# penn-pal-lab/robot_aware_control

Hardware: AMD Instinct MI355X
Metric: SVG train frames/sec + CEM candidate-rollouts/sec, 64x64 (higher is better)
Workload: dtype fp32 (conv operands as two fp16 parts = 22 significant bits, fp32 accumulate; see fp32_exact)

## Files before the change

include/rac_hip.h:

```cpp
#ifndef RAC_HIP_H
#define RAC_HIP_H

#include <stddef.h>
#include <stdint.h>

#ifdef __cplusplus
extern "C" {
#endif

#define RAC_OK 0
#define RAC_EINVAL (-1)
#define RAC_ELAUNCH (-2)

#define RAC_ABI_VERSION 12

int rac_version(void);
const char* rac_device_arch(void);
const char* rac_last_error(void);

enum {
  RAC_CONV_FWD = 0,
  RAC_CONV_DGRAD = 1,
  RAC_CONV_WGRAD = 2
};
// ... 169 lines not shown
int rac_reparam_head_bwd(const rac_grad_src* dz_srcs, int32_t n_srcs, const float* logvar, const float* eps,
                         const float* dmu_add, const float* dlogvar_add, float* dy, int64_t M, int32_t z,
                         uint32_t* dy_amax, void* stream);

int rac_reparam_fwd(const float* mu, const float* logvar, const float* eps, float* z, int64_t n, void* stream);
int rac_reparam_bwd(const float* dz, const float* logvar, const float* eps, float* dlogvar, int64_t n, void* stream);

int rac_pack_input(const float* img, const float* zmask, const float* mask, int32_t Cm, int32_t pad, float* packed,
                   int32_t B, int32_t HW, void* stream);
int rac_first_layer_fwd(const float* img, const float* zmask, const float* mask, int32_t Cm, const float* w,
                        const float* scale, const float* shift, int32_t act, float* out, uint32_t* out_amax,
                        int32_t amax_per_image, int32_t B, int32_t H, int32_t W, int32_t Cout, void* stream);
int rac_first_layer_fwd_split(const float* img, const float* zmask, const float* mask, int32_t Cm, const float* w,
                              const float* scale, const float* shift, int32_t act, float* out, uint32_t* out_amax,
                              int32_t amax_per_image, int32_t B, int32_t H, int32_t W, int32_t Cout, void* stream);
int rac_head_fwd(const float* x, const float* w_taps, const float* bias, float* y, int32_t B, int32_t H, int32_t W,
                 void* stream);
int rac_head_dgrad(const float* d, const float* w, float* dx, int32_t B, int32_t H, int32_t W, void* stream);
int rac_head_fwd_split(const float* x, const uint32_t* x_amax, int32_t amax_per_image, const float* w_taps,
                       const float* bias, float* y, int32_t B, int32_t H, int32_t W, void* stream);
int rac_thin_wgrad(const float* wide, const float* thin, int32_t thin_stride, int32_t Ct, float* parts, int32_t n_parts,
                   int32_t B, int32_t H, int32_t W, int32_t Cw, void* stream);
int rac_unpack_grad(const float* dpacked, int32_t C, const float* zmask, float* dimg, int32_t B, int32_t HW,
                    void* stream);
int rac_zero_region(const float* img, const float* mask, float* out, int32_t B, int32_t HW, void* stream);
int rac_composite_fwd(const float* x4, const float* prev, float* out, int32_t B, int32_t HW, void* stream);
int rac_composite_bwd(const float* dout, const float* x4, const float* prev, float* dx4, float* dprev, int32_t B,
                      int32_t HW, void* stream);
int rac_predict_frames(const float* x4, const float* prev, const float* target, const float* true_mask, float* pred,
                       uint8_t* gen_u8, uint8_t* true_u8, int64_t image_stride, int32_t n, int32_t nt, int32_t H,
                       int32_t W, void* stream);

typedef struct rac_image_job {
  int64_t frame_offset, mask_offset;
  int32_t Hs, Ws, top, left, th, tw;
  int32_t order[4];
  int32_t jitter;
// ... 135 lines not shown
```

robot_aware_control_amd/_lib.py:

```python
from __future__ import annotations

import ctypes as C
import os

import torch

_HERE = os.path.dirname(os.path.abspath(__file__))
LIB_PATH = os.environ.get("RAC_HIP_LIB") or os.path.join(_HERE, "librac_hip.so")

i32, i64, f32, vp = C.c_int32, C.c_int64, C.c_float, C.c_void_p


class ConvArgs(C.Structure):
    _fields_ = [
        ("mode", i32), ("B", i32), ("H", i32), ("W", i32), ("ksize", i32), ("Cin", i32), ("Cout", i32),
        ("act", i32), ("split_k", i32), ("accumulate", i32), ("a_split", i32), ("o_split", i32),
        ("slab_stride", i64),
        ("a0", vp), ("a1", vp), ("w", vp), ("out0", vp), ("out1", vp),
        ("bias", vp), ("scale", vp), ("shift", vp), ("stats", vp),
        ("stats_rows", i64), ("a0_up", i32), ("amax_per_image", i32),
    ]


WGRAD_MAX_STEPS = 16
# ... 104 lines not shown
    "rac_groupnorm_fwd": [vp, vp, vp, vp, vp, vp, i32, i32, i32, i32, f32, vp],
    "rac_norm_lstm_cell_fwd": [vp, vp, vp, vp, vp, vp, vp, vp, vp, vp, vp, vp, vp, vp, vp, vp, i32, i32, i32, f32, vp],
    "rac_groupnorm_bwd": [vp, vp, vp, vp, vp, vp, vp, vp, i32, i32, i32, i32, vp],
    "rac_norm_lstm_cell_bwd": [vp] * 25 + [i32, i32, i32, vp],
    "rac_lstm_out_fwd": [vp, vp, vp, i64, i32, vp],
    "rac_lstm_out_bwd": [vp, vp, vp, vp, vp, i64, i32, vp],
    "rac_lstm_core_bwd": [vp, vp, vp, vp, vp, vp, i64, i32, vp],
    "rac_grad_sum": [C.POINTER(GradSrc), i32, vp, i64, i32, vp, vp],
    "rac_lstm_cell_bwd_srcs": [C.POINTER(GradSrc), i32, vp, vp, vp, vp, vp, vp, i64, i32, vp, vp],
    "rac_reparam_head_bwd": [C.POINTER(GradSrc), i32, vp, vp, vp, vp, vp, i64, i32, vp, vp],
    "rac_reparam_fwd": [vp, vp, vp, vp, i64, vp],
    "rac_reparam_bwd": [vp, vp, vp, vp, i64, vp],
    "rac_pack_input": [vp, vp, vp, i32, i32, vp, i32, i32, vp],
    "rac_first_layer_fwd": [vp, vp, vp, i32, vp, vp, vp, i32, vp, vp, i32, i32, i32, i32, i32, vp],
    "rac_first_layer_fwd_split": [vp, vp, vp, i32, vp, vp, vp, i32, vp, vp, i32, i32, i32, i32, i32, vp],
    "rac_head_fwd": [vp, vp, vp, vp, i32, i32, i32, vp],
    "rac_head_dgrad": [vp, vp, vp, i32, i32, i32, vp],
    "rac_head_fwd_split": [vp, vp, i32, vp, vp, vp, i32, i32, i32, vp],
    "rac_thin_wgrad": [vp, vp, i32, i32, vp, i32, i32, i32, i32, i32, vp],
    "rac_unpack_grad": [vp, i32, vp, vp, i32, i32, vp],
    "rac_zero_region": [vp, vp, vp, i32, i32, vp],
    "rac_composite_fwd": [vp, vp, vp, i32, i32, vp],
    "rac_composite_bwd": [vp, vp, vp, vp, vp, i32, i32, vp],
    "rac_predict_frames": [vp, vp, vp, vp, vp, vp, vp, i64, i32, i32, i32, i32, vp],
    "rac_image_job_bytes": [],
    "rac_image_pipeline": [vp, vp, vp, vp, vp, i32, i32, i32, i32, vp],
    "rac_det_pack_fwd": [vp, i32, vp, i32, vp, vp, vp, i32, vp, vp, vp, i32, i32, i32, vp, vp],
    "rac_det_pack_bwd": [vp, i32, i32, vp, i32, vp, i32, vp, vp, vp, vp, vp, i32, i32, vp],
    "rac_copy_baseline": [vp, vp, vp, vp, i32, i32, vp],
    "rac_recon_loss_fwd": [i32, vp, vp, vp, f32, vp, vp, vp, i32, i32, vp],
    "rac_recon_loss_bwd": [i32, vp, vp, vp, f32, vp, vp, vp, vp, i32, i32, vp],
    "rac_kl_fwd": [vp, vp, vp, vp, i64, i32, vp, vp, vp],
    "rac_kl_bwd": [vp, vp, vp, vp, vp, i64, i32, vp, vp, vp, vp, vp],
    "rac_psnr_ssim": [vp, vp, vp, vp, vp, vp, i32, i32, i32, vp],
# ... 83 lines not shown
```

robot_aware_control_amd/csrc/rac_frame.hip:

```cpp
#include "rac_common.h"

namespace rac {

static inline int grid_for(long work_items) {
  long b = (work_items + 255) / 256;
  return (int)(b < 1 ? 1 : (b > 2048 ? 2048 : b));
}

__global__ void pack_input_kernel(const float* img, const float* zmask, const float* mask, int Cm, int pad,
                                  float* packed, int B, int HW) {
  const int C = 3 + Cm + pad;
  const long n = (long)B * HW;
  for (long i = blockIdx.x * (long)blockDim.x + threadIdx.x; i < n; i += (long)gridDim.x * blockDim.x) {
    long b = i / HW;
    int p = (int)(i - b * HW);
    const bool zero = zmask && zmask[i] != 0.f;
    float* o = packed + i * C;
#pragma unroll
    for (int c = 0; c < 3; ++c) {
      float v = img[(b * 3 + c) * HW + p];
      o[c] = zero ? v * 0.f : v;
    }
    for (int c = 0; c < Cm; ++c) o[3 + c] = mask[(b * Cm + c) * HW + p];
    for (int c = 0; c < pad; ++c) o[3 + Cm + c] = 0.f;
// ... 112 lines not shown
      for (int c4 = 0; c4 < 8; ++c4) {
        const f32x4 xv = *reinterpret_cast<const f32x4*>(xp + c4 * 4);
#pragma unroll
        for (int j = 0; j < 4; ++j)
#pragma unroll
          for (int c = 0; c < 4; ++c) acc[c] += xv[j] * wp[(c4 * 4 + j) * 4 + c];
      }
    }
  }
  f32x4 out;
#pragma unroll
  for (int c = 0; c < 4; ++c) out[c] = sigmoid_acc(acc[c]);
  *reinterpret_cast<f32x4*>(y + (((long)b * H + ty0 + py) * W + tx0 + px) * 4) = out;
}

template <int CT>
__global__ __launch_bounds__(256) void thin_wgrad_kernel(const float* wide, const float* thin, int ldt, float* part, int H,
                                                         int W, int n_tiles) {
  constexpr int TP = 18, NO = 9 * CT, NQ = (NO + 3) / 4;
  __shared__ float th[TP * TP][CT];
  const int tid = threadIdx.x, w = tid & 63, q = tid >> 6;
  const int tiles_x = W >> 4, tiles_img = (H >> 4) * tiles_x;
  float acc[NQ];
  int toff[NQ];
#pragma unroll
  for (int j = 0; j < NQ; ++j) {
    acc[j] = 0.f;
    const int o = min(q * NQ + j, NO - 1), tap = o / CT;
    toff[j] = ((tap / 3) * TP + tap % 3) * CT + (o - tap * CT);
  }
  const float* thf = &th[0][0];
  for (int tile = blockIdx.x; tile < n_tiles; tile += gridDim.x) {
    const int b = tile / tiles_img, ti = tile - b * tiles_img;
    const int ty0 = (ti / tiles_x) << 4, tx0 = (ti % tiles_x) << 4;
    __syncthreads();
    for (int i = tid; i < TP * TP * CT; i += 256) {
      const int pix = i / CT, t = i - pix * CT;
      const int y = ty0 + pix / TP - 1, x = tx0 + pix % TP - 1;
      th[pix][t] = ((unsigned)y < (unsigned)H && (unsigned)x < (unsigned)W)
                       ? thin[(((long)b * H + y) * W + x) * ldt + t] : 0.f;
    }
    __syncthreads();
    const float* wp = wide + (((long)b * H + ty0) * W + tx0) * 64 + w;
    for (int py = 0; py < 16; ++py) {
      float v[16];
#pragma unroll
      for (int px = 0; px < 16; ++px) v[px] = wp[((long)py * W + px) * 64];
#pragma unroll
      for (int px = 0; px < 16; ++px) {
        const float* tp = thf + (py * TP + px) * CT;
#pragma unroll
        for (int j = 0; j < NQ; ++j) acc[j] += v[px] * tp[toff[j]];
      }
    }
  }
  float* dst = part + (long)blockIdx.x * 64 * NO + (long)w * NO;
#pragma unroll
  for (int j = 0; j < NQ; ++j) {
    const int o = q * NQ + j;
    if (o < NO) dst[o] = acc[j];
  }
}

__global__ void unpack_grad_kernel(const float* dpacked, int C, const float* zmask, float* dimg, int B, int HW) {
  const long n = (long)B * HW;
  for (long i = blockIdx.x * (long)blockDim.x + threadIdx.x; i < n; i += (long)gridDim.x * blockDim.x) {
    long b = i / HW;
    int p = (int)(i - b * HW);
    const bool zero = zmask && zmask[i] != 0.f;
#pragma unroll
    for (int c = 0; c < 3; ++c) dimg[(b * 3 + c) * HW + p] = zero ? 0.f : dpacked[i * C + c];
  }
}

__global__ void zero_region_kernel(const float* img, const float* mask, float* out, int B, int HW) {
// ... 157 lines not shown
    }
  }
}

__device__ __forceinline__ float block_sum(float v, float* sh) {
  v = wave_sum(v);
  const int w = threadIdx.x >> 6, l = threadIdx.x & 63;
  __syncthreads();
  if (l == 0) sh[w] = v;
  __syncthreads();
  float t = 0.f;
  for (int k = 0; k < (int)(blockDim.x >> 6); ++k) t += sh[k];
  return t;
}

__global__ void recon_loss_sample_kernel(int kind, const float* pred, const float* target, const float* mask,
                                         float rw, float* per_sample, int HW) {
  __shared__ float sh[16];
  const int b = blockIdx.x;
  const long base = (long)b * 3 * HW;
  float s_main = 0.f, s_world_n = 0.f, s_rob2 = 0.f, s_rob_n = 0.f, s_world2 = 0.f;
  for (int p = threadIdx.x; p < HW; p += blockDim.x) {
    const bool rob = mask && mask[(long)b * HW + p] != 0.f;
    if (mask) {
      if (rob) s_rob_n += 3.f; else s_world_n += 3.f;
    }
#pragma unroll
    for (int c = 0; c < 3; ++c) {
      float d = target[base + (long)c * HW + p] - pred[base + (long)c * HW + p];
      if (mask) {
        if (rob) s_rob2 += d * d; else s_world2 += d * d;
      }
// ... 288 lines not shown
  RAC_REQUIRE(W % 16 == 0 && aligned16(d) && aligned16(w) && aligned16(dx), "rac_head_dgrad: W % 16 == 0, 16-byte aligned buffers");
  const long n_pix = (long)B * H * W;
  long per_block = ((n_pix + 511) / 512 + 15) / 16 * 16;
  if (per_block < 64) per_block = 64;
  const long blocks = (n_pix + per_block - 1) / per_block;
  RAC_REQUIRE(blocks < (1L << 31) && per_block < (1L << 31) && n_pix < (1L << 28) - 16, "rac_head_dgrad: too many pixels");
  hipLaunchKernelGGL(head_dgrad_kernel, dim3((unsigned)blocks), dim3(256), 0, ST(stream), reinterpret_cast<const float4*>(d),
                     reinterpret_cast<const float4*>(w), reinterpret_cast<float4*>(dx), H, W, n_pix, (int)per_block);
  return check_launch("rac_head_dgrad");
}

int rac_thin_wgrad(const float* wide, const float* thin, int32_t thin_stride, int32_t Ct, float* parts, int32_t n_parts,
                   int32_t B, int32_t H, int32_t W, int32_t Cw, void* stream) {
  RAC_REQUIRE(wide && thin && parts && B > 0 && H > 0 && W > 0 && Ct >= 1 && Ct <= 8 && thin_stride >= Ct && n_parts >= 1,
              "rac_thin_wgrad: bad args (1 <= Ct <= 8)");
  RAC_REQUIRE(Cw == 64 && H % 16 == 0 && W % 16 == 0, "rac_thin_wgrad: Cw 64, H and W multiples of 16");
  const int n_tiles = B * (H / 16) * (W / 16);
  RAC_REQUIRE(n_parts <= n_tiles, "rac_thin_wgrad: more parts than 16 x 16 tiles");
  typedef void (*fn_t)(const float*, const float*, int, float*, int, int, int);
  static const fn_t fns[8] = {thin_wgrad_kernel<1>, thin_wgrad_kernel<2>, thin_wgrad_kernel<3>, thin_wgrad_kernel<4>,
                              thin_wgrad_kernel<5>, thin_wgrad_kernel<6>, thin_wgrad_kernel<7>, thin_wgrad_kernel<8>};
  hipLaunchKernelGGL(fns[Ct - 1], dim3(n_parts), dim3(256), 0, ST(stream), wide, thin, thin_stride, parts, H, W, n_tiles);
  return check_launch("rac_thin_wgrad");
}

int rac_unpack_grad(const float* dpacked, int32_t C, const float* zmask, float* dimg, int32_t B, int32_t HW,
                    void* stream) {
  RAC_REQUIRE(dpacked && dimg && C >= 3 && B > 0 && HW > 0, "rac_unpack_grad: bad args");
  hipLaunchKernelGGL(unpack_grad_kernel, dim3(grid_for((long)B * HW)), dim3(256), 0, ST(stream), dpacked, C, zmask,
                     dimg, B, HW);
  return check_launch("rac_unpack_grad");
}

int rac_zero_region(const float* img, const float* mask, float* out, int32_t B, int32_t HW, void* stream) {
  RAC_REQUIRE(img && mask && out && B > 0 && HW > 0, "rac_zero_region: bad args");
  hipLaunchKernelGGL(zero_region_kernel, dim3(grid_for((long)B * 3 * HW)), dim3(256), 0, ST(stream), img, mask, out, B,
                     HW);
  return check_launch("rac_zero_region");
// ... 46 lines not shown
                  (!sheet || (aligned4(sheet) && aligned4(start_u8) && aligned4(goal_u8) && aligned4(goal_mask))),
              "rac_cem_rollout_sheet: 16-byte aligned float buffers, strides multiples of 4, 4-byte aligned uint8 buffers");
  const long quads = (long)(T + 1) * R * H * (W / 4);
  RAC_REQUIRE((long)H * W < (1L << 29) && quads < (1L << 40), "rac_cem_rollout_sheet: too many pixels");
  hipLaunchKernelGGL(cem_rollout_sheet_kernel, dim3(grid_for(quads)), dim3(256), 0, ST(stream), frames, (long)step_stride,
                     (long)cand_stride, rows, R, T, start_u8, goal_u8, G, goal_mask, obs, sheet, H, W);
  return check_launch("rac_cem_rollout_sheet");
}

int rac_recon_loss_fwd(int32_t kind, const float* pred, const float* target, const float* mask, float robot_weight,
                       const float* batch_weight, float* per_sample, float* out, int32_t B, int32_t HW, void* stream) {
  RAC_REQUIRE(kind >= 0 && kind <= 3 && pred && target && per_sample && out && B > 0 && HW > 0,
              "rac_recon_loss_fwd: bad args");
  RAC_REQUIRE(!((kind == RAC_LOSS_DONTCARE_L1 || kind == RAC_LOSS_DONTCARE_MSE) && !mask),
              "rac_recon_loss_fwd: dontcare loss needs a mask");
  hipLaunchKernelGGL(recon_loss_sample_kernel, dim3(B), dim3(256), 0, ST(stream), kind, pred, target, mask,
                     robot_weight, per_sample, HW);
  hipLaunchKernelGGL(recon_loss_final_kernel, dim3(1), dim3(256), 0, ST(stream), kind, per_sample, batch_weight,
                     mask != nullptr, out, B, HW);
  return check_launch("rac_recon_loss_fwd");
}

int rac_recon_loss_bwd(int32_t kind, const float* pred, const float* target, const float* mask, float robot_weight,
                       const float* batch_weight, const float* per_sample, const float* gout, float* dpred, int32_t B,
                       int32_t HW, void* stream) {
  RAC_REQUIRE(kind >= 0 && kind <= 3 && pred && target && per_sample && gout && dpred && B > 0 && HW > 0,
              "rac_recon_loss_bwd: bad args");
  RAC_REQUIRE(!((kind == RAC_LOSS_DONTCARE_L1 || kind == RAC_LOSS_DONTCARE_MSE) && !mask),
              "rac_recon_loss_bwd: dontcare loss needs a mask");
  hipLaunchKernelGGL(recon_loss_bwd_kernel, dim3(grid_for((long)B * 3 * HW)), dim3(256), 0, ST(stream), kind, pred,
                     target, mask, robot_weight, batch_weight, per_sample, gout, dpred, B, HW);
// ... 546 lines not shown
```

robot_aware_control_amd/csrc/rac_split16.hip:

```cpp
#include <math.h>
#include <stdlib.h>

#include <type_traits>

#include "rac_common.h"

namespace rac {

typedef _Float16 f16x8 __attribute__((ext_vector_type(8)));
typedef _Float16 f16x4 __attribute__((ext_vector_type(4)));
typedef unsigned int u32x4 __attribute__((ext_vector_type(4)));
typedef unsigned int u32x2 __attribute__((ext_vector_type(2)));
typedef __amdgpu_buffer_rsrc_t rsrc_t;

constexpr unsigned OOB = 0xFFFFFFF0u;
constexpr int SBN = 128, SBK = 32;

__device__ __forceinline__ const void* uniform_ptr(const void* p) {
  unsigned long long v = reinterpret_cast<unsigned long long>(p);
  unsigned lo = __builtin_amdgcn_readfirstlane((unsigned)v);
  unsigned hi = __builtin_amdgcn_readfirstlane((unsigned)(v >> 32));
  return reinterpret_cast<const void*>(((unsigned long long)hi << 32) | lo);
}
__device__ __forceinline__ rsrc_t make_rsrc(const void* p, unsigned bytes) {
// ... 707 lines not shown
    {
      const int py = tid >> 4, px = tid & 15;
      f32x4 o = b4;
#pragma unroll
      for (int tap = 0; tap < 9; ++tap) {
        const int ky = tap / 3, kx = tap - ky * 3;
        o += *reinterpret_cast<const f32x4*>(zs + (tap * H16_ZS + (py + 2 - ky) * H16_P + px + 2 - kx) * 4);
      }
#pragma unroll
      for (int c = 0; c < 4; ++c) o[c] = sigmoid_acc(o[c]);
      *reinterpret_cast<f32x4*>(y + (((long)b * H + ty0 + py) * W + tx0 + px) * 4) = o;
    }
  }
}

template <int CIN>
__global__ __launch_bounds__(256, 2) void first16_kernel(const float* __restrict__ img, const float* __restrict__ zmask,
                                                         const float* __restrict__ mask, const float* __restrict__ w,
                                                         const float* __restrict__ scale, const float* __restrict__ shift,
                                                         int act, float* __restrict__ out, unsigned* amax, int per_image,
                                                         int H, int W, int n_tiles) {
  constexpr int KK = 9 * CIN, KS = (KK + 31) / 32, TP = 18, TPW = 20, PL = TP * TPW;
  __shared__ float in_sh[CIN * PL];
  const int tid = threadIdx.x, lane = tid & 63, lr = lane & 15, lq = lane >> 4;
  const int wid = __builtin_amdgcn_readfirstlane(tid >> 6);
  f16x8 fw[4][KS][2];
  float osc[4][4], osh[4][4];
#pragma unroll
  for (int j = 0; j < 4; ++j) {
    const float* wr = w + (long)(16 * j + lr) * KK;
    float wv[KS][8], mx = 0.f;
#pragma unroll
    for (int s = 0; s < KS; ++s)
#pragma unroll
      for (int i = 0; i < 8; ++i) {
        const int k = 32 * s + 8 * lq + i;
        const float t = wr[min(k, KK - 1)];
        wv[s][i] = k < KK ? t : 0.f;
// ... 4 lines not shown
    const int kw = scale_exp(__builtin_bit_cast(unsigned, mx));
    const float sw = pow2f(kw);
#pragma unroll
    for (int s = 0; s < KS; ++s)
#pragma unroll
      for (int i = 0; i < 8; ++i) {
        const float v = wv[s][i] * sw;
        const _Float16 a = (_Float16)v;
        fw[j][s][0][i] = a;
        fw[j][s][1][i] = (_Float16)(v - (float)a);
      }
#pragma unroll
    for (int r = 0; r < 4; ++r) {
      const int kwr = __shfl(kw, 4 * lq + r);
      const int co = 16 * j + 4 * lq + r;
      osc[j][r] = (scale ? scale[co] : 1.f) * pow2f(-kwr);
      osh[j][r] = scale ? shift[co] : 0.f;
    }
  }
  int goff[KS][8];
#pragma unroll
  for (int s = 0; s < KS; ++s)
#pragma unroll
    for (int i = 0; i < 8; ++i) {
      const int k = min(32 * s + 8 * lq + i, KK - 1), tap = k / CIN, ci = k - tap * CIN;
      goff[s][i] = ci * PL + (tap / 3) * TPW + tap % 3;
    }
  const float slope = act == RAC_ACT_LEAKY02 ? 0.2f : 1.f;
  const int tiles_x = W >> 4, tiles_img = (H >> 4) * tiles_x;
  const long HW = (long)H * W;

  constexpr int NST = (CIN * TP * TP + 255) / 256;
// ... 58 lines not shown
        for (int i = 0; i < 8; ++i) {
          const float v = xv[s][i] * sa;
          const _Float16 a = (_Float16)v;
          fx[s][0][i] = a;
          fx[s][1][i] = (_Float16)(v - (float)a);
        }
      float* op = out + (((long)b * H + ty0 + py) * W + tx0 + lr) * 64 + 4 * lq;
#pragma unroll
      for (int j = 0; j < 4; ++j) {
        f32x4 acc = {0.f, 0.f, 0.f, 0.f};
#pragma unroll
        for (int s = 0; s < KS; ++s) acc = mma3(fw[j][s], fx[s], acc);
        f32x4 o;
#pragma unroll
        for (int r = 0; r < 4; ++r) {
          float v = fmaf(acc[r] * ia, osc[j][r], osh[j][r]);
          v = v > 0.f ? v : slope * v;
          mxo = max(mxo, absbits(v));
          o[r] = v;
        }
        *reinterpret_cast<f32x4*>(op + 16 * j) = o;
      }
    }
    if (amax) amax_commit_block(mxo, per_image ? amax + b : amax);
  }
}

template <int NV, int WM, int NT, int D, bool FAST = false, int KSF = 3>
__global__ __launch_bounds__(256, 2) void conv16_rows_kernel(Conv16P p) {
  constexpr int PF = KSF / 2, TAPSF = KSF * KSF;
  constexpr int WN = 4 / WM;
  constexpr int MB = 8 / WM;
  constexpr int NB = 2 * NT;
  constexpr int BNW = WN * NT * 32;
  extern __shared__ __attribute__((aligned(16))) unsigned char lds_raw[];
  const int tid = threadIdx.x;
  const int lane = tid & 63;
  const int wid = __builtin_amdgcn_readfirstlane(tid >> 6);
  const int lr = lane & 15, lq = lane >> 4;
// ... 1719 lines not shown
}

extern "C" int rac_first_layer_fwd_split(const float* img, const float* zmask, const float* mask, int32_t Cm, const float* w,
                                         const float* scale, const float* shift, int32_t act, float* out,
                                         uint32_t* out_amax, int32_t amax_per_image, int32_t B, int32_t H, int32_t W,
                                         int32_t Cout, void* stream) {
  RAC_REQUIRE(img && w && out && B > 0 && H > 0 && W > 0 && Cm >= 0 && Cm <= 5 && (Cm == 0 || mask),
              "rac_first_layer_fwd_split: bad args (3 image planes + at most 5 mask / heatmap planes)");
  RAC_REQUIRE(Cout == 64 && H % 16 == 0 && W % 16 == 0 && (scale == nullptr) == (shift == nullptr) && aligned16(out) &&
                  (act == RAC_ACT_NONE || act == RAC_ACT_LEAKY02),
              "rac_first_layer_fwd_split: Cout 64, H and W multiples of 16, act none / leaky");
  const long n_tiles = (long)B * (H / 16) * (W / 16);
  RAC_REQUIRE(n_tiles < (1L << 31), "rac_first_layer_fwd_split: too many tiles");
  const int grid = (int)(n_tiles < 1024 ? n_tiles : 1024);
  typedef void (*fn_t)(const float*, const float*, const float*, const float*, const float*, const float*, int, float*,
                       unsigned*, int, int, int, int);
  static const fn_t fns[6] = {first16_kernel<3>, first16_kernel<4>, first16_kernel<5>,
                              first16_kernel<6>, first16_kernel<7>, first16_kernel<8>};
  hipLaunchKernelGGL(fns[Cm], dim3(grid), dim3(256), 0, reinterpret_cast<hipStream_t>(stream), img, zmask, mask, w, scale,
                     shift, act, out, out_amax, amax_per_image ? 1 : 0, H, W, (int)n_tiles);
  return check_launch("rac_first_layer_fwd_split");
}

extern "C" int rac_head_fwd_split(const float* x, const uint32_t* x_amax, int32_t amax_per_image, const float* w_taps,
                                  const float* bias, float* y, int32_t B, int32_t H, int32_t W, void* stream) {
  RAC_REQUIRE(x && x_amax && w_taps && bias && y && B > 0 && H > 0 && W > 0, "rac_head_fwd_split: bad args");
  RAC_REQUIRE(H % 16 == 0 && W % 16 == 0 && aligned16(x) && aligned16(y) && aligned16(bias),
              "rac_head_fwd_split: H % 16 == 0, W % 16 == 0, 16-byte aligned buffers");
  RAC_REQUIRE((long)H * W * 64 * 4 < (1L << 32), "rac_head_fwd_split: image too large for one buffer descriptor");
  const long n_tiles = (long)B * (H / 16) * (W / 16);
  RAC_REQUIRE(n_tiles < (1L << 31), "rac_head_fwd_split: too many tiles");
  const int grid = (int)(n_tiles < 768 ? n_tiles : 768);
  hipLaunchKernelGGL(head16_kernel, dim3(grid), dim3(256), 0, reinterpret_cast<hipStream_t>(stream), x, x_amax,
                     amax_per_image, w_taps, bias, y, H, W, (int)n_tiles);
  return check_launch("rac_head_fwd_split");
}
// ... 116 lines not shown
```

robot_aware_control_amd/ops.py:

```python
from __future__ import annotations

import contextlib
import ctypes as C
import functools
import os
import weakref
from typing import Optional, Tuple

import torch

from . import _lib
from ._lib import (AbsmaxJob, AdamFragJob, AdamRange, ConvArgs, FragJob, GradSrc, OptimRange, WgradArgs, call, ptr,
                   stream_ptr)

FWD, DGRAD, WGRAD = 0, 1, 2
ACT_NONE, ACT_LEAKY, ACT_SIGMOID = 0, 1, 2
LOSS_KINDS = {"mse": 0, "l1": 1, "dontcare_mse": 2, "dontcare_l1": 3}
BN_EPS, BN_MOMENTUM = 1e-5, 0.1


def _require_cuda(t: torch.Tensor):
    if not t.is_cuda:
        raise _lib.RacError("robot_aware_control_amd ops run on the GPU only (no CPU fallback); got a CPU tensor")

# ... 67 lines not shown
        if ent is not None:
            ent.tag = None
        return wp
    return _derived(weight, f"_rac_padded{cp}", build)


def wgrad_padded_acc(dy, x0, weight):
    co, ci, k, _ = weight.shape
    cp = x0.shape[3]
    gp = torch.zeros((co, k, k, cp), device=dy.device, dtype=torch.float32).permute(0, 3, 1, 2)
    B, H, W, Cout = dy.shape
    conv_raw(WGRAD, x0, None, dy, gp, B=B, H=H, W=W, ksize=k, Cin=cp, Cout=Cout, a_split=cp, accumulate=1, split_k=0)
    call("rac_unpad_add", ptr(gp), cp, ptr(weight_mem(grad_buffer(weight))), ci, co * k * k, stream_ptr())


def thin_wgrad_acc(wide, thin, ct: int, weight):
    B, H, W, _ = wide.shape
    n = 64 * 9 * ct
    n_parts = min(512, B * (H // 16) * (W // 16))
    parts = torch.empty((n_parts, n), device=wide.device, dtype=torch.float32)
    sp = stream_ptr()
    call("rac_thin_wgrad", ptr(wide), ptr(thin), thin.shape[3], ct, ptr(parts), n_parts, B, H, W, 64, sp)
    call("rac_slab_accumulate", ptr(parts), n_parts, n, ptr(weight_mem(grad_buffer(weight))), n, sp)


MAX_SPLIT_K = int(os.environ.get("RAC_MAX_SPLIT_K", "8"))


def plan_split_k(M: int, N: int, nchunks: int, tile128_only: bool = False) -> int:
    return _plan_split_k(M, N, nchunks, tile128_only, os.environ.get("RAC_SPLIT"), MAX_SPLIT_K)


@functools.lru_cache(maxsize=None)
def _plan_split_k(M, N, nchunks, tile128_only, forced, max_split):
# ... 1382 lines not shown
                    thin_wgrad_acc(draw, x0, weight.shape[1], weight)
                elif split:
                    conv_wgrad_split_acc(draw, x0, x1, weight)
                elif padded:
                    wgrad_padded_acc(draw, x0, weight)
                else:
                    conv_wgrad_acc(draw, x0, x1, weight)
            if _WINDOW is not None and _WINDOW.vgg_steps and split and not padded and wgrad_split_ok(x0, x1, weight):
                conv_wgrad_split_acc(draw, x0, x1, weight, defer=True)
            else:
                wgrad_on_side_stream(wgrad, (draw, x0, x1), need_amax=split)
        return dx0, dx1, None, None, None, None, None, None, None, None, None


FIRST_TRAIN_MFMA = os.environ.get("RAC_FIRST_TRAIN_MFMA", "1") == "1"


class FirstVggLayer(torch.autograd.Function):

    @staticmethod
    def forward(ctx, img, zero_mask, mask, weight, gamma, beta, rmean, rvar, n_updates, groups):
        B, _, H, W = img.shape
        Cm = mask.shape[1] if mask is not None else 0
        dev = img.device
        raw = torch.empty((B, H, W, 64), device=dev, dtype=torch.float32)
        sp = stream_ptr()
        call("rac_first_layer_fwd_split", ptr(img), ptr(zero_mask), ptr(mask), Cm, ptr(weight_mem(weight.detach())), None,
             None, ACT_NONE, ptr(raw), None, 0, B, H, W, 64, sp)
        G = int(groups)
        M = B * H * W
        stats = zeros64((G, 2, 64), dev)
        call("rac_col_stats", ptr(raw), ptr(stats), M, 64, G, sp)
        y, aff = bn_apply_act(raw, stats, gamma, beta, rmean, rvar, n_updates, M, 64, G)
        ctx.save_for_backward(img, zero_mask, mask, weight, gamma, beta, raw, aff)
        ctx.groups = G
        return y

    @staticmethod
    def backward(ctx, dy):
        img, zero_mask, mask, weight, gamma, beta, raw, aff = ctx.saved_tensors
        dy = dy.contiguous()
        B, H, W, _ = raw.shape
        M, G = B * H * W, ctx.groups
        sp = stream_ptr()
        sums = zeros64((G, 2, 64), dy.device)
        call("rac_bn_bwd_reduce", ptr(dy), ptr(raw), ptr(aff[0]), ptr(aff[1]), ptr(aff[2]), ptr(aff[3]), ptr(sums), M, 64, G,
             sp)
        draw = torch.empty_like(raw)
        want_affine = gamma.requires_grad
        call("rac_bn_bwd_apply", ptr(dy), ptr(raw), ptr(aff[0]), ptr(aff[1]), ptr(aff[2]), ptr(aff[3]), ptr(sums), ptr(draw),
             ptr(grad_buffer(gamma)) if want_affine else None, ptr(grad_buffer(beta)) if want_affine else None, M, 64, G,
             None, sp)
        if weight.requires_grad:
            Cm = mask.shape[1] if mask is not None else 0
            pad = pad4(3 + Cm)
            x0 = torch.empty((B, H, W, 3 + Cm + pad), device=dy.device, dtype=torch.float32)
            call("rac_pack_input", ptr(img), ptr(zero_mask), ptr(mask), Cm, pad, ptr(x0), B, H * W, sp)
            thin_wgrad_acc(draw, x0, 3 + Cm, weight)
        return (None,) * 10


def first_layer_train_ok(img, mask, weight) -> bool:
    return (FIRST_TRAIN_MFMA and FIRST_MFMA and SPLIT_GEMM and not img.requires_grad and first_layer_ok(img, mask, weight)
            and img.shape[0] * (img.shape[-2] // 16) * (img.shape[-1] // 16) > 0)


def vgg_pool_frozen(x0, weight, scale, shift):
    Cout = weight.shape[0]
    if not (SPLIT_GEMM and Cout >= SPLIT_MIN_COUT and x0.shape[3] == weight.shape[1] and x0.shape[1] % 2 == 0
# ... 1438 lines not shown
```

Baseline: 4214.

## Fuse first-layer BN stats into forward conv and BN backward into thin wgrad

```diff
diff --git a/include/rac_hip.h b/include/rac_hip.h
--- a/include/rac_hip.h
+++ b/include/rac_hip.h
@@ -207,6 +207,9 @@
 int rac_first_layer_fwd_split(const float* img, const float* zmask, const float* mask, int32_t Cm, const float* w,
                               const float* scale, const float* shift, int32_t act, float* out, uint32_t* out_amax,
                               int32_t amax_per_image, int32_t B, int32_t H, int32_t W, int32_t Cout, void* stream);
+int rac_first_layer_fwd_stats(const float* img, const float* zmask, const float* mask, int32_t Cm, const float* w,
+                              float* out, double* stats, int32_t groups, int32_t B, int32_t H, int32_t W, int32_t Cout,
+                              void* stream);
 int rac_head_fwd(const float* x, const float* w_taps, const float* bias, float* y, int32_t B, int32_t H, int32_t W,
                  void* stream);
 int rac_head_dgrad(const float* d, const float* w, float* dx, int32_t B, int32_t H, int32_t W, void* stream);
@@ -214,6 +217,10 @@
                        const float* bias, float* y, int32_t B, int32_t H, int32_t W, void* stream);
 int rac_thin_wgrad(const float* wide, const float* thin, int32_t thin_stride, int32_t Ct, float* parts, int32_t n_parts,
                    int32_t B, int32_t H, int32_t W, int32_t Cw, void* stream);
+int rac_first_layer_bwd(const float* dy, const float* raw, const float* scale, const float* shift, const float* mean,
+                        const float* invstd, const double* sums, const float* img, const float* zmask, const float* mask,
+                        int32_t Cm, float* parts, int32_t n_parts, float* dgamma, float* dbeta, int32_t B, int32_t H,
+                        int32_t W, int32_t groups, void* stream);
 int rac_unpack_grad(const float* dpacked, int32_t C, const float* zmask, float* dimg, int32_t B, int32_t HW,
                     void* stream);
 int rac_zero_region(const float* img, const float* mask, float* out, int32_t B, int32_t HW, void* stream);
diff --git a/robot_aware_control_amd/_lib.py b/robot_aware_control_amd/_lib.py
--- a/robot_aware_control_amd/_lib.py
+++ b/robot_aware_control_amd/_lib.py
@@ -142,10 +142,12 @@
     "rac_pack_input": [vp, vp, vp, i32, i32, vp, i32, i32, vp],
     "rac_first_layer_fwd": [vp, vp, vp, i32, vp, vp, vp, i32, vp, vp, i32, i32, i32, i32, i32, vp],
     "rac_first_layer_fwd_split": [vp, vp, vp, i32, vp, vp, vp, i32, vp, vp, i32, i32, i32, i32, i32, vp],
+    "rac_first_layer_fwd_stats": [vp, vp, vp, i32, vp, vp, vp, i32, i32, i32, i32, i32, vp],
     "rac_head_fwd": [vp, vp, vp, vp, i32, i32, i32, vp],
     "rac_head_dgrad": [vp, vp, vp, i32, i32, i32, vp],
     "rac_head_fwd_split": [vp, vp, i32, vp, vp, vp, i32, i32, i32, vp],
     "rac_thin_wgrad": [vp, vp, i32, i32, vp, i32, i32, i32, i32, i32, vp],
+    "rac_first_layer_bwd": [vp, vp, vp, vp, vp, vp, vp, vp, vp, vp, i32, vp, i32, vp, vp, i32, i32, i32, i32, vp],
     "rac_unpack_grad": [vp, i32, vp, vp, i32, i32, vp],
     "rac_zero_region": [vp, vp, vp, i32, i32, vp],
     "rac_composite_fwd": [vp, vp, vp, i32, i32, vp],
diff --git a/robot_aware_control_amd/csrc/rac_frame.hip b/robot_aware_control_amd/csrc/rac_frame.hip
--- a/robot_aware_control_amd/csrc/rac_frame.hip
+++ b/robot_aware_control_amd/csrc/rac_frame.hip
@@ -150,51 +150,147 @@
   *reinterpret_cast<f32x4*>(y + (((long)b * H + ty0 + py) * W + tx0 + px) * 4) = out;
 }
 
-template <int CT>
-__global__ __launch_bounds__(256) void thin_wgrad_kernel(const float* wide, const float* thin, int ldt, float* part, int H,
-                                                         int W, int n_tiles) {
+struct ThinWgradP {
+  const float* wide;
+  const float* thin;
+  int ldt;
+  const float *raw, *scale, *shift, *mean, *invstd;
+  const double* sums;
+  const float *img, *zmask, *mask;
+  float *part, *dgamma, *dbeta;
+  int H, W, n_tiles, imgs_per_group, G;
+};
+
+template <int CT, bool FUSED>
+__global__ __launch_bounds__(256) void thin_wgrad_kernel(ThinWgradP p) {
   constexpr int TP = 18, NO = 9 * CT, NQ = (NO + 3) / 4;
-  __shared__ float th[TP * TP][CT];
-  const int tid = threadIdx.x, w = tid & 63, q = tid >> 6;
+  __shared__ float th[TP * TP * CT];
+  const int tid = threadIdx.x, lane = tid & 63, c4 = lane & 15, ps = lane >> 4;
+  const int q = __builtin_amdgcn_readfirstlane(tid >> 6);
+  const int H = p.H, W = p.W;
   const int tiles_x = W >> 4, tiles_img = (H >> 4) * tiles_x;
-  float acc[NQ];
+  f32x4 acc[NQ];
   int toff[NQ];
 #pragma unroll
   for (int j = 0; j < NQ; ++j) {
-    acc[j] = 0.f;
+    acc[j] = f32x4{0.f, 0.f, 0.f, 0.f};
     const int o = min(q * NQ + j, NO - 1), tap = o / CT;
-    toff[j] = ((tap / 3) * TP + tap % 3) * CT + (o - tap * CT);
-  }
-  const float* thf = &th[0][0];
-  for (int tile = blockIdx.x; tile < n_tiles; tile += gridDim.x) {
+    toff[j] = ((tap / 3) * TP + tap % 3 + ps) * CT + (o - tap * CT);
+  }
+  const long HW = (long)H * W;
+  for (int tile = blockIdx.x; tile < p.n_tiles; tile += gridDim.x) {
     const int b = tile / tiles_img, ti = tile - b * tiles_img;
     const int ty0 = (ti / tiles_x) << 4, tx0 = (ti % tiles_x) << 4;
     __syncthreads();
-    for (int i = tid; i < TP * TP * CT; i += 256) {
-      const int pix = i / CT, t = i - pix * CT;
-      const int y = ty0 + pix / TP - 1, x = tx0 + pix % TP - 1;
-      th[pix][t] = ((unsigned)y < (unsigned)H && (unsigned)x < (unsigned)W)
-                       ? thin[(((long)b * H + y) * W + x) * ldt + t] : 0.f;
+    if (FUSED) {
+      for (int i = tid; i < TP * TP * CT; i += 256) {
+        const int t = i / (TP * TP), pix = i - t * TP * TP;
+        const int y = ty0 + pix / TP - 1, x = tx0 + pix % TP - 1;
+        float v = 0.f;
+        if ((unsigned)y < (unsigned)H && (unsigned)x < (unsigned)W) {
+          const long px = (long)y * W + x;
+          if (t < 3) {
+            v = p.img[((long)b * 3 + t) * HW + px];
+            if (p.zmask && p.zmask[(long)b * HW + px] != 0.f) v = v * 0.f;
+          } else {
+            v = p.mask[((long)b * (CT - 3) + (t - 3)) * HW + px];
+          }
+        }
+        th[pix * CT + t] = v;
+      }
+    } else {
+      for (int i = tid; i < TP * TP * CT; i += 256) {
+        const int pix = i / CT, t = i - pix * CT;
+        const int y = ty0 + pix / TP - 1, x = tx0 + pix % TP - 1;
+        th[i] = ((unsigned)y < (unsigned)H && (unsigned)x < (unsigned)W)
+                    ? p.thin[(((long)b * H + y) * W + x) * p.ldt + t] : 0.f;
+      }
     }
     __syncthreads();
-    const float* wp = wide + (((long)b * H + ty0) * W + tx0) * 64 + w;
+    f32x4 sc, sh, mu, is, m1, m2;
+    if (FUSED) {
+      const int g = b / p.imgs_per_group;
+      const double invM = 1.0 / ((double)p.imgs_per_group * (double)HW);
+      const double* sg = p.sums + (long)g * 128;
+#pragma unroll
+      for (int e = 0; e < 4; ++e) {
+        const int c = 4 * c4 + e, gc = g * 64 + c;
+        sc[e] = p.scale[gc], sh[e] = p.shift[gc], mu[e] = p.mean[gc], is[e] = p.invstd[gc];
+        m1[e] = (float)(sg[c] * invM), m2[e] = (float)(sg[64 + c] * invM);
+      }
+    }
+    const long base = ((((long)b * H + ty0) * W + tx0 + ps) << 6) + 4 * c4;
+    const float* wp = p.wide + base;
+    const float* rp = FUSED ? p.raw + base : nullptr;
+    f32x4 v[4], r[4];
+#pragma unroll
+    for (int s = 0; s < 4; ++s) {
+      v[s] = *reinterpret_cast<const f32x4*>(wp + (s << 8));
+      if (FUSED) r[s] = *reinterpret_cast<const f32x4*>(rp + (s << 8));
+    }
+#pragma unroll 2
     for (int py = 0; py < 16; ++py) {
-      float v[16];
-#pragma unroll
-      for (int px = 0; px < 16; ++px) v[px] = wp[((long)py * W + px) * 64];
-#pragma unroll
-      for (int px = 0; px < 16; ++px) {
-        const float* tp = thf + (py * TP + px) * CT;
-#pragma unroll
-        for (int j = 0; j < NQ; ++j) acc[j] += v[px] * tp[toff[j]];
-      }
-    }
-  }
-  float* dst = part + (long)blockIdx.x * 64 * NO + (long)w * NO;
-#pragma unroll
-  for (int j = 0; j < NQ; ++j) {
-    const int o = q * NQ + j;
-    if (o < NO) dst[o] = acc[j];
+      f32x4 vn[4], rn[4];
+      const long nrow = ((long)min(py + 1, 15) * W) << 6;
+#pragma unroll
+      for (int s = 0; s < 4; ++s) {
+        vn[s] = *reinterpret_cast<const f32x4*>(wp + nrow + (s << 8));
+        if (FUSED) rn[s] = *reinterpret_cast<const f32x4*>(rp + nrow + (s << 8));
+      }
+      const float* tr = th + py * TP * CT;
+#pragma unroll
+      for (int s = 0; s < 4; ++s) {
+        f32x4 d = v[s];
+        if (FUSED) {
+#pragma unroll
+          for (int e = 0; e < 4; ++e) {
+            const float xv = r[s][e];
+            const float z = xv * sc[e] + sh[e];
+            const float dz = d[e] * (z > 0.f ? 1.f : 0.2f);
+            const float xh = (xv - mu[e]) * is[e];
+            d[e] = sc[e] * (dz - m1[e] - xh * m2[e]);
+          }
+        }
+#pragma unroll
+        for (int j = 0; j < NQ; ++j) acc[j] += d * tr[toff[j] + 4 * s * CT];
+      }
+#pragma unroll
+      for (int s = 0; s < 4; ++s) {
+        v[s] = vn[s];
+        if (FUSED) r[s] = rn[s];
+      }
+    }
+  }
+#pragma unroll
+  for (int j = 0; j < NQ; ++j)
+#pragma unroll
+    for (int e = 0; e < 4; ++e) {
+      float a = acc[j][e];
+      a += __shfl_xor(a, 16);
+      a += __shfl_xor(a, 32);
+      acc[j][e] = a;
+    }
+  if (ps == 0) {
+    float* dst = p.part + (long)blockIdx.x * 64 * NO + (long)(4 * c4) * NO;
+#pragma unroll
+    for (int j = 0; j < NQ; ++j) {
+      const int o = q * NQ + j;
+      if (o < NO) {
+#pragma unroll
+        for (int e = 0; e < 4; ++e) dst[e * NO + o] = acc[j][e];
+      }
+    }
+  }
+  if (FUSED && blockIdx.x == 0 && p.dgamma) {
+    for (int c = tid; c < 64; c += 256) {
+      double a = 0., bsum = 0.;
+      for (int g = 0; g < p.G; ++g) {
+        a += p.sums[(long)g * 128 + 64 + c];
+        bsum += p.sums[(long)g * 128 + c];
+      }
+      p.dgamma[c] += (float)a;
+      p.dbeta[c] += (float)bsum;
+    }
   }
 }
 
@@ -382,8 +478,8 @@
   return t;
 }
 
-__global__ void recon_loss_sample_kernel(int kind, const float* pred, const float* target, const float* mask,
-                                         float rw, float* per_sample, int HW) {
+__global__ __launch_bounds__(1024) void recon_loss_sample_kernel(int kind, const float* pred, const float* target,
+                                                                 const float* mask, float rw, float* per_sample, int HW) {
   __shared__ float sh[16];
   const int b = blockIdx.x;
   const long base = (long)b * 3 * HW;
@@ -702,14 +798,43 @@
                    int32_t B, int32_t H, int32_t W, int32_t Cw, void* stream) {
   RAC_REQUIRE(wide && thin && parts && B > 0 && H > 0 && W > 0 && Ct >= 1 && Ct <= 8 && thin_stride >= Ct && n_parts >= 1,
               "rac_thin_wgrad: bad args (1 <= Ct <= 8)");
-  RAC_REQUIRE(Cw == 64 && H % 16 == 0 && W % 16 == 0, "rac_thin_wgrad: Cw 64, H and W multiples of 16");
-  const int n_tiles = B * (H / 16) * (W / 16);
+  RAC_REQUIRE(Cw == 64 && H % 16 == 0 && W % 16 == 0 && aligned16(wide),
+              "rac_thin_wgrad: Cw 64, H and W multiples of 16, 16-byte aligned wide");
+  const long n_tiles = (long)B * (H / 16) * (W / 16);
+  RAC_REQUIRE(n_tiles < (1L << 31), "rac_thin_wgrad: too many tiles");
   RAC_REQUIRE(n_parts <= n_tiles, "rac_thin_wgrad: more parts than 16 x 16 tiles");
-  typedef void (*fn_t)(const float*, const float*, int, float*, int, int, int);
-  static const fn_t fns[8] = {thin_wgrad_kernel<1>, thin_wgrad_kernel<2>, thin_wgrad_kernel<3>, thin_wgrad_kernel<4>,
-                              thin_wgrad_kernel<5>, thin_wgrad_kernel<6>, thin_wgrad_kernel<7>, thin_wgrad_kernel<8>};
-  hipLaunchKernelGGL(fns[Ct - 1], dim3(n_parts), dim3(256), 0, ST(stream), wide, thin, thin_stride, parts, H, W, n_tiles);
+  ThinWgradP p{};
+  p.wide = wide, p.thin = thin, p.ldt = thin_stride, p.part = parts, p.H = H, p.W = W, p.n_tiles = (int)n_tiles;
+  typedef void (*fn_t)(ThinWgradP);
+  static const fn_t fns[8] = {thin_wgrad_kernel<1, false>, thin_wgrad_kernel<2, false>, thin_wgrad_kernel<3, false>,
+                              thin_wgrad_kernel<4, false>, thin_wgrad_kernel<5, false>, thin_wgrad_kernel<6, false>,
+                              thin_wgrad_kernel<7, false>, thin_wgrad_kernel<8, false>};
+  hipLaunchKernelGGL(fns[Ct - 1], dim3(n_parts), dim3(256), 0, ST(stream), p);
   return check_launch("rac_thin_wgrad");
+}
+
+int rac_first_layer_bwd(const float* dy, const float* raw, const float* scale, const float* shift, const float* mean,
+                        const float* invstd, const double* sums, const float* img, const float* zmask, const float* mask,
+                        int32_t Cm, float* parts, int32_t n_parts, float* dgamma, float* dbeta, int32_t B, int32_t H,
+                        int32_t W, int32_t groups, void* stream) {
+  RAC_REQUIRE(dy && raw && scale && shift && mean && invstd && sums && img && parts && B > 0 && H > 0 && W > 0 && Cm >= 0 &&
+                  Cm <= 5 && (Cm == 0 || mask) && n_parts >= 1 && groups >= 1 && B % groups == 0,
+              "rac_first_layer_bwd: bad args (3 image planes + at most 5 mask planes, whole images per group)");
+  RAC_REQUIRE((dgamma == nullptr) == (dbeta == nullptr), "rac_first_layer_bwd: dgamma/dbeta must come together");
+  RAC_REQUIRE(H % 16 == 0 && W % 16 == 0 && aligned16(dy) && aligned16(raw),
+              "rac_first_layer_bwd: H and W multiples of 16, 16-byte aligned dy / raw");
+  const long n_tiles = (long)B * (H / 16) * (W / 16);
+  RAC_REQUIRE(n_tiles < (1L << 31), "rac_first_layer_bwd: too many tiles");
+  RAC_REQUIRE(n_parts <= n_tiles, "rac_first_layer_bwd: more parts than 16 x 16 tiles");
+  ThinWgradP p{};
+  p.wide = dy, p.raw = raw, p.scale = scale, p.shift = shift, p.mean = mean, p.invstd = invstd, p.sums = sums;
+  p.img = img, p.zmask = zmask, p.mask = mask, p.part = parts, p.dgamma = dgamma, p.dbeta = dbeta;
+  p.H = H, p.W = W, p.n_tiles = (int)n_tiles, p.imgs_per_group = B / groups, p.G = groups;
+  typedef void (*fn_t)(ThinWgradP);
+  static const fn_t fns[6] = {thin_wgrad_kernel<3, true>, thin_wgrad_kernel<4, true>, thin_wgrad_kernel<5, true>,
+                              thin_wgrad_kernel<6, true>, thin_wgrad_kernel<7, true>, thin_wgrad_kernel<8, true>};
+  hipLaunchKernelGGL(fns[Cm], dim3(n_parts), dim3(256), 0, ST(stream), p);
+  return check_launch("rac_first_layer_bwd");
 }
 
 int rac_unpack_grad(const float* dpacked, int32_t C, const float* zmask, float* dimg, int32_t B, int32_t HW,
@@ -786,7 +911,7 @@
               "rac_recon_loss_fwd: bad args");
   RAC_REQUIRE(!((kind == RAC_LOSS_DONTCARE_L1 || kind == RAC_LOSS_DONTCARE_MSE) && !mask),
               "rac_recon_loss_fwd: dontcare loss needs a mask");
-  hipLaunchKernelGGL(recon_loss_sample_kernel, dim3(B), dim3(256), 0, ST(stream), kind, pred, target, mask,
+  hipLaunchKernelGGL(recon_loss_sample_kernel, dim3(B), dim3(1024), 0, ST(stream), kind, pred, target, mask,
                      robot_weight, per_sample, HW);
   hipLaunchKernelGGL(recon_loss_final_kernel, dim3(1), dim3(256), 0, ST(stream), kind, per_sample, batch_weight,
                      mask != nullptr, out, B, HW);
diff --git a/robot_aware_control_amd/csrc/rac_split16.hip b/robot_aware_control_amd/csrc/rac_split16.hip
--- a/robot_aware_control_amd/csrc/rac_split16.hip
+++ b/robot_aware_control_amd/csrc/rac_split16.hip
@@ -745,14 +745,16 @@
   }
 }
 
-template <int CIN>
+template <int CIN, bool STATS = false>
 __global__ __launch_bounds__(256, 2) void first16_kernel(const float* __restrict__ img, const float* __restrict__ zmask,
                                                          const float* __restrict__ mask, const float* __restrict__ w,
                                                          const float* __restrict__ scale, const float* __restrict__ shift,
                                                          int act, float* __restrict__ out, unsigned* amax, int per_image,
-                                                         int H, int W, int n_tiles) {
+                                                         int H, int W, int n_tiles, double* stats = nullptr,
+                                                         int imgs_per_group = 1) {
   constexpr int KK = 9 * CIN, KS = (KK + 31) / 32, TP = 18, TPW = 20, PL = TP * TPW;
   __shared__ float in_sh[CIN * PL];
+  __shared__ __attribute__((aligned(16))) float st_sh[STATS ? 8 * 256 * 4 : 4];
   const int tid = threadIdx.x, lane = tid & 63, lr = lane & 15, lq = lane >> 4;
   const int wid = __builtin_amdgcn_readfirstlane(tid >> 6);
   f16x8 fw[4][KS][2];
@@ -787,8 +789,8 @@
     for (int r = 0; r < 4; ++r) {
       const int kwr = __shfl(kw, 4 * lq + r);
       const int co = 16 * j + 4 * lq + r;
-      osc[j][r] = (scale ? scale[co] : 1.f) * pow2f(-kwr);
-      osh[j][r] = scale ? shift[co] : 0.f;
+      osc[j][r] = (!STATS && scale ? scale[co] : 1.f) * pow2f(-kwr);
+      osh[j][r] = !STATS && scale ? shift[co] : 0.f;
     }
   }
   int goff[KS][8];
@@ -877,15 +879,42 @@
         f32x4 o;
 #pragma unroll
         for (int r = 0; r < 4; ++r) {
-          float v = fmaf(acc[r] * ia, osc[j][r], osh[j][r]);
-          v = v > 0.f ? v : slope * v;
-          mxo = max(mxo, absbits(v));
+          float v;
+          if (STATS) {
+            v = acc[r] * ia * osc[j][r];
+          } else {
+            v = fmaf(acc[r] * ia, osc[j][r], osh[j][r]);
+            v = v > 0.f ? v : slope * v;
+            mxo = max(mxo, absbits(v));
+          }
           o[r] = v;
         }
         *reinterpret_cast<f32x4*>(op + 16 * j) = o;
-      }
-    }
-    if (amax) amax_commit_block(mxo, per_image ? amax + b : amax);
+        if (STATS) {
+          f32x4* sp = reinterpret_cast<f32x4*>(st_sh) + j * 256 + tid;
+          if (n == 0) {
+            sp[0] = o, sp[1024] = o * o;
+          } else {
+            sp[0] += o, sp[1024] += o * o;
+          }
+        }
+      }
+    }
+    if (STATS) {
+      __syncthreads();
+      const int o = tid >> 1, hf = tid & 1, i = o >> 2, q4 = o & 3;
+      const float* rp = st_sh + (((i >> 2) * 256 + hf * 128 + q4 * 16) << 2) + (i & 3);
+      float t = 0.f;
+#pragma unroll
+      for (int w2 = 0; w2 < 2; ++w2)
+#pragma unroll
+        for (int l = 0; l < 16; ++l) t += rp[(w2 * 64 + l) << 2];
+      t += __shfl_xor(t, 1);
+      if (hf == 0)
+        atomicAdd(stats + (long)(b / imgs_per_group) * 128 + (i >> 4) * 64 + 16 * ((i >> 2) & 3) + 4 * q4 + (i & 3), (double)t);
+    } else if (amax) {
+      amax_commit_block(mxo, per_image ? amax + b : amax);
+    }
   }
 }
 
@@ -2635,12 +2664,33 @@
   RAC_REQUIRE(n_tiles < (1L << 31), "rac_first_layer_fwd_split: too many tiles");
   const int grid = (int)(n_tiles < 1024 ? n_tiles : 1024);
   typedef void (*fn_t)(const float*, const float*, const float*, const float*, const float*, const float*, int, float*,
-                       unsigned*, int, int, int, int);
+                       unsigned*, int, int, int, int, double*, int);
   static const fn_t fns[6] = {first16_kernel<3>, first16_kernel<4>, first16_kernel<5>,
                               first16_kernel<6>, first16_kernel<7>, first16_kernel<8>};
   hipLaunchKernelGGL(fns[Cm], dim3(grid), dim3(256), 0, reinterpret_cast<hipStream_t>(stream), img, zmask, mask, w, scale,
-                     shift, act, out, out_amax, amax_per_image ? 1 : 0, H, W, (int)n_tiles);
+                     shift, act, out, out_amax, amax_per_image ? 1 : 0, H, W, (int)n_tiles, (double*)nullptr, 1);
   return check_launch("rac_first_layer_fwd_split");
+}
+
+extern "C" int rac_first_layer_fwd_stats(const float* img, const float* zmask, const float* mask, int32_t Cm, const float* w,
+                                         float* out, double* stats, int32_t groups, int32_t B, int32_t H, int32_t W,
+                                         int32_t Cout, void* stream) {
+  RAC_REQUIRE(img && w && out && stats && B > 0 && H > 0 && W > 0 && Cm >= 0 && Cm <= 5 && (Cm == 0 || mask) && groups >= 1 &&
+                  B % groups == 0,
+              "rac_first_layer_fwd_stats: bad args (3 image planes + at most 5 mask planes, whole images per group)");
+  RAC_REQUIRE(Cout == 64 && H % 16 == 0 && W % 16 == 0 && aligned16(out),
+              "rac_first_layer_fwd_stats: Cout 64, H and W multiples of 16");
+  const long n_tiles = (long)B * (H / 16) * (W / 16);
+  RAC_REQUIRE(n_tiles < (1L << 31), "rac_first_layer_fwd_stats: too many tiles");
+  const int grid = (int)(n_tiles < 1024 ? n_tiles : 1024);
+  typedef void (*fn_t)(const float*, const float*, const float*, const float*, const float*, const float*, int, float*,
+                       unsigned*, int, int, int, int, double*, int);
+  static const fn_t fns[6] = {first16_kernel<3, true>, first16_kernel<4, true>, first16_kernel<5, true>,
+                              first16_kernel<6, true>, first16_kernel<7, true>, first16_kernel<8, true>};
+  hipLaunchKernelGGL(fns[Cm], dim3(grid), dim3(256), 0, reinterpret_cast<hipStream_t>(stream), img, zmask, mask, w,
+                     (const float*)nullptr, (const float*)nullptr, (int)RAC_ACT_NONE, out, (unsigned*)nullptr, 0, H, W,
+                     (int)n_tiles, stats, B / groups);
+  return check_launch("rac_first_layer_fwd_stats");
 }
 
 extern "C" int rac_head_fwd_split(const float* x, const uint32_t* x_amax, int32_t amax_per_image, const float* w_taps,
diff --git a/robot_aware_control_amd/ops.py b/robot_aware_control_amd/ops.py
--- a/robot_aware_control_amd/ops.py
+++ b/robot_aware_control_amd/ops.py
@@ -105,10 +105,14 @@
     call("rac_unpad_add", ptr(gp), cp, ptr(weight_mem(grad_buffer(weight))), ci, co * k * k, stream_ptr())
 
 
+def thin_wgrad_parts(B: int, H: int, W: int) -> int:
+    return min(512, B * (H // 16) * (W // 16))
+
+
 def thin_wgrad_acc(wide, thin, ct: int, weight):
     B, H, W, _ = wide.shape
     n = 64 * 9 * ct
-    n_parts = min(512, B * (H // 16) * (W // 16))
+    n_parts = thin_wgrad_parts(B, H, W)
     parts = torch.empty((n_parts, n), device=wide.device, dtype=torch.float32)
     sp = stream_ptr()
     call("rac_thin_wgrad", ptr(wide), ptr(thin), thin.shape[3], ct, ptr(parts), n_parts, B, H, W, 64, sp)
@@ -1521,6 +1525,8 @@
 
 
 FIRST_TRAIN_MFMA = os.environ.get("RAC_FIRST_TRAIN_MFMA", "1") == "1"
+FIRST_FWD_STATS = os.environ.get("RAC_FIRST_FWD_STATS", "1") == "1"
+FIRST_BWD_FUSED = os.environ.get("RAC_FIRST_BWD_FUSED", "1") == "1"
 
 
 class FirstVggLayer(torch.autograd.Function):
@@ -1532,12 +1538,16 @@
         dev = img.device
         raw = torch.empty((B, H, W, 64), device=dev, dtype=torch.float32)
         sp = stream_ptr()
-        call("rac_first_layer_fwd_split", ptr(img), ptr(zero_mask), ptr(mask), Cm, ptr(weight_mem(weight.detach())), None,
-             None, ACT_NONE, ptr(raw), None, 0, B, H, W, 64, sp)
         G = int(groups)
         M = B * H * W
         stats = zeros64((G, 2, 64), dev)
-        call("rac_col_stats", ptr(raw), ptr(stats), M, 64, G, sp)
+        if FIRST_FWD_STATS and B % G == 0:
+            call("rac_first_layer_fwd_stats", ptr(img), ptr(zero_mask), ptr(mask), Cm, ptr(weight_mem(weight.detach())),
+                 ptr(raw), ptr(stats), G, B, H, W, 64, sp)
+        else:
+            call("rac_first_layer_fwd_split", ptr(img), ptr(zero_mask), ptr(mask), Cm, ptr(weight_mem(weight.detach())), None,
+                 None, ACT_NONE, ptr(raw), None, 0, B, H, W, 64, sp)
+            call("rac_col_stats", ptr(raw), ptr(stats), M, 64, G, sp)
         y, aff = bn_apply_act(raw, stats, gamma, beta, rmean, rvar, n_updates, M, 64, G)
         ctx.save_for_backward(img, zero_mask, mask, weight, gamma, beta, raw, aff)
         ctx.groups = G
@@ -1553,13 +1563,22 @@
         sums = zeros64((G, 2, 64), dy.device)
         call("rac_bn_bwd_reduce", ptr(dy), ptr(raw), ptr(aff[0]), ptr(aff[1]), ptr(aff[2]), ptr(aff[3]), ptr(sums), M, 64, G,
              sp)
+        want_affine = gamma.requires_grad
+        dgamma = ptr(grad_buffer(gamma)) if want_affine else None
+        dbeta = ptr(grad_buffer(beta)) if want_affine else None
+        Cm = mask.shape[1] if mask is not None else 0
+        if FIRST_BWD_FUSED and weight.requires_grad and B % G == 0:
+            n = 64 * 9 * (3 + Cm)
+            n_parts = thin_wgrad_parts(B, H, W)
+            parts = torch.empty((n_parts, n), device=dy.device, dtype=torch.float32)
+            call("rac_first_layer_bwd", ptr(dy), ptr(raw), ptr(aff[0]), ptr(aff[1]), ptr(aff[2]), ptr(aff[3]), ptr(sums),
+                 ptr(img), ptr(zero_mask), ptr(mask), Cm, ptr(parts), n_parts, dgamma, dbeta, B, H, W, G, sp)
+            call("rac_slab_accumulate", ptr(parts), n_parts, n, ptr(weight_mem(grad_buffer(weight))), n, sp)
+            return (None,) * 10
         draw = torch.empty_like(raw)
-        want_affine = gamma.requires_grad
         call("rac_bn_bwd_apply", ptr(dy), ptr(raw), ptr(aff[0]), ptr(aff[1]), ptr(aff[2]), ptr(aff[3]), ptr(sums), ptr(draw),
-             ptr(grad_buffer(gamma)) if want_affine else None, ptr(grad_buffer(beta)) if want_affine else None, M, 64, G,
-             None, sp)
+             dgamma, dbeta, M, 64, G, None, sp)
         if weight.requires_grad:
-            Cm = mask.shape[1] if mask is not None else 0
             pad = pad4(3 + Cm)
             x0 = torch.empty((B, H, W, 3 + Cm + pad), device=dy.device, dtype=torch.float32)
             call("rac_pack_input", ptr(img), ptr(zero_mask), ptr(mask), Cm, pad, ptr(x0), B, H * W, sp)
```

Result: no change. 4254, median of 6 (+1.0%).
